# bifurcationkit/BifurcationKit.jl

Measured on NVIDIA H100. Metric: continuation steps/sec (SH2d PALC), higher is better.
Workload: dtype f64

## Files before the change

### bifurcationkit.jl_b200/csrc/bk_common.cuh

```cuda
#pragma once
#include <cuda_runtime.h>
#include <stdint.h>
#include <stdlib.h>
#include <string>
#include <unordered_map>
#include <vector>
#include "../../include/bk200.h"
#include <nvtx3/nvToolsExt.h>

struct BkRange {
  explicit BkRange(const char* name) { nvtxRangePushA(name); }
  ~BkRange() { nvtxRangePop(); }
};

#define BK_MAX_PAR 8
#define BK_NSM_FALLBACK 132

struct OpDesc {
  int kind;
  int nx, ny, nz;
  double cx, cy, cz;
  double par[BK_MAX_PAR];
  const double* u;
  double a0, a1;
// ... 76 lines not shown
      cudaEvent_t a, b;
      cudaEventCreate(&a);
      cudaEventCreate(&b);
      pairs.push_back({a, b});
    }
    cudaEventRecord(pairs[used++].first, st);
  }
  void end(cudaStream_t st) { cudaEventRecord(pairs[used - 1].second, st); }
  long long harvest(double& ms) {
    long long k = 0;
    for (size_t i = 0; i < used; ++i) {
      float t = 0;
      if (cudaEventElapsedTime(&t, pairs[i].first, pairs[i].second) == cudaSuccess) {
        ms += t;
        ++k;
      }
    }
    used = 0;
    return k;
  }
  void destroy() {
    for (auto& p : pairs) {
      cudaEventDestroy(p.first);
      cudaEventDestroy(p.second);
    }
    pairs.clear();
    used = 0;
  }
};

struct bk_ctx {
  int device = 0;
  int nsm = BK_NSM_FALLBACK;
  cudaStream_t stream = nullptr;
  int kind = 0;
  long long dims[3] = {1, 1, 1};
  double lengths[3] = {1, 1, 1};
  double par[BK_MAX_PAR] = {0};
  long long N = 0;
  long long N0 = 0;
  bool cplx = false;
  double shift_imag = 0;
  bool transpose = false;
  int m = 0;
  long long ld = 0;
  double* u_state = nullptr;
  double jpar[BK_MAX_PAR] = {0};
  bool have_state = false;
  double* phi = nullptr;
  double* xpi = nullptr;
  double* fcache = nullptr;
  double phi_dot_xpi = 0;
  double* V = nullptr;
  double* w = nullptr;
  double* z = nullptr;
  double* r = nullptr;
  double* scales = nullptr;
  double* gcoef = nullptr;
  double* hcols = nullptr;
  double* hcols2 = nullptr;
  double* h_pinned = nullptr;
  double* partials = nullptr;
  int gmax = 0;
  unsigned int* counters = nullptr;
  double* red_out = nullptr;
  double* red_pinned = nullptr;
// ... 54 lines not shown
  return g < c->gmax ? g : c->gmax;
}
static inline double bk_inv_h2(const bk_ctx* c, int d) {
  const double h = 2 * c->lengths[d] / c->dims[d];
  return 1.0 / (h * h);
}

bool bk_is_device_ptr(const void* p);
int bk_stage_in(bk_ctx* c, const double* p, long long n, int slot, bool copy_in, double** dev);
int bk_stage_out(bk_ctx* c, double* p, long long n, const double* dev);

OpDesc bk_make_op(bk_ctx* c, double a0, double a1);
OpDesc bk_make_residual_op(bk_ctx* c);
int bk_launch_residual(bk_ctx* c, const double* u_dev, double* out_dev);
int bk_launch_apply(bk_ctx* c, const OpDesc& op, const double* in_dev, const double* in_scale_ptr, double* out_dev);
int bk_potrap_refresh_cache(bk_ctx* c);

int bk_precond_apply_dev(bk_ctx* c, const double* in_dev, double* out_dev, long long n);

int bk_periodic_setup(bk_ctx* c);
int bk_periodic_residual(bk_ctx* c, const OpDesc& op, const double* u, double* out);
int bk_periodic_jvp(bk_ctx* c, const OpDesc& op, const double* in, const double* sp, double* out);
int bk_periodic_fused(bk_ctx* c, const OpDesc& op, const double* in, const double* sp, double* out, bool left);

int bk_dev_axpby(bk_ctx* c, double* y, double a, const double* x, double b, long long n);
int bk_dev_scale(bk_ctx* c, double* x, double a, long long n);
int bk_dev_dot(bk_ctx* c, const double* x, const double* y, long long n, double* out_host);
int bk_dev_norminf(bk_ctx* c, const double* x, long long n, double* out_host);
int bk_dev_copy(bk_ctx* c, double* dst, const double* src, long long n);

int bk_gmres_dev(bk_ctx* c, const OpDesc& op, const double* rhs_dev, double* x_dev, const bk_gmres_opts* o,
                 int* converged, int* iters, double* resnorm);
int bk_launch_dots(bk_ctx* c, const double* basis, const double* scales, const double* w, long long n, int j, double* hcol,
                   double* gcoef);
int bk_launch_update(bk_ctx* c, const double* basis, const double* gcoef, const double* w, long long n, int j, double* vout,
                     double* h_out, double* scale_out);
int bk_launch_lincomb(bk_ctx* c, const double* basis, const double* scales, double* x, double beta, long long n, int k,
                      const double* coef_dev);
int bk_tmp(bk_ctx* c, int slot, double** out);

void bk_grant_smem(int device, const void* kern, size_t bytes);
template <typename K>
static inline void bk_ensure_smem(bk_ctx* c, K kern, size_t bytes) {
  size_t& cur = c->smem_attr[(const void*)kern];
  if (bytes > cur) {
    bk_grant_smem(c->device, (const void*)kern, bytes);
    cur = bytes;
  }
}

#ifdef __CUDACC__
template <typename... KArgs, typename... Args>
static inline cudaError_t bk_launch_pdl(void (*kern)(KArgs...), dim3 grid, dim3 block, size_t smem, cudaStream_t st, bool pdl,
                                        Args&&... args) {
  cudaLaunchConfig_t cfg = {};
  cfg.gridDim = grid;
  cfg.blockDim = block;
  cfg.dynamicSmemBytes = smem;
  cfg.stream = st;
  cudaLaunchAttribute at[1];
  at[0].id = cudaLaunchAttributeProgrammaticStreamSerialization;
  at[0].val.programmaticStreamSerializationAllowed = 1;
  cfg.attrs = at;
  static int no_pdl = -1;
  if (no_pdl < 0) no_pdl = getenv("BK_NO_PDL") ? 1 : 0;
  cfg.numAttrs = pdl && !no_pdl ? 1 : 0;
  return cudaLaunchKernelEx(&cfg, kern, KArgs(args)...);
}
template <typename... KArgs, typename... Args>
// ... 89 lines not shown
```

### bifurcationkit.jl_b200/csrc/bk_ctx.cu

```cuda
#include <cstdio>
#include <cstring>
#include <map>
#include <mutex>
#include <new>
#include "bk_common.cuh"

int bk_fail(bk_ctx* c, int code, const char* what, const char* file, int line) {
  if (c) {
    char buf[512];
    snprintf(buf, sizeof buf, "%s (%s:%d)", what, file, line);
    c->err = buf;
  }
  return code;
}

void bk_grant_smem(int device, const void* kern, size_t bytes) {
  static std::mutex mu;
  static std::map<std::pair<int, const void*>, size_t> granted;
  std::lock_guard<std::mutex> lk(mu);
  size_t& cur = granted[{device, kern}];
  if (bytes <= cur) return;
  cudaFuncSetAttribute(kern, cudaFuncAttributeMaxDynamicSharedMemorySize, (int)bytes);
  if (bytes > 48 * 1024) cudaFuncSetAttribute(kern, cudaFuncAttributePreferredSharedMemoryCarveout, 100);
  cur = bytes;
// ... 63 lines not shown
  if (!c) return BK_ERR_ARG;
  *out = c;
  c->device = device;
  c->cplx = (kind & BK_COMPLEX) != 0;
  kind &= ~BK_COMPLEX;
  c->kind = kind;
  for (int i = 0; i < 3; ++i) {
    c->dims[i] = dims ? (dims[i] > 0 ? dims[i] : 1) : 1;
    c->lengths[i] = lengths ? lengths[i] : 1.0;
  }
  const BkKindTraits* kt = bk_kind_traits(kind);
  if (!kt) return bk_fail(c, BK_ERR_ARG, "unknown problem kind", __FILE__, __LINE__);
  if (kt->pow2_grid)
    for (int d = 0; d < 2; ++d) {
      const long long v = c->dims[d];
      BK_CHECK(c, v >= 64 && v <= 2048 && (v & (v - 1)) == 0,
               "BK_SH2D_PERIODIC: Nx and Ny must be powers of two from 64 to 2048");
    }
  long long n = kt->fields;
  for (int d = 0; d < kt->ndims; ++d) n *= c->dims[d];
  n += kt->extra;
  BK_CHECK(c, n >= 2, "problem too small");
  BK_CHECK(c, krylov_m >= 1 && krylov_m <= 1024, "krylov_m out of range");
  BK_CHECK(c, !c->cplx || kt->complex_ok, "BK_COMPLEX is not available for the periodic-orbit functional");
  c->N0 = n;
  if (c->cplx) n *= 2;
  c->N = n;
  c->m = krylov_m;
  c->ld = ((n + 2 + 31) / 32) * 32;
  BK_CUDA(c, cudaSetDevice(device));
  cudaDeviceProp prop;
  BK_CUDA(c, cudaGetDeviceProperties(&prop, device));
  c->nsm = prop.multiProcessorCount;
  if (const char* e = getenv("BK_NSM")) {
    const int v = atoi(e);
    if (v >= 1 && v <= 1024) c->nsm = v;
  }
  BK_CUDA(c, cudaStreamCreateWithFlags(&c->stream, cudaStreamNonBlocking));
  size_t ld = (size_t)c->ld, m = (size_t)c->m;
  BK_CUDA(c, cudaMalloc(&c->u_state, 8 * ld));
  BK_CUDA(c, cudaMalloc(&c->V, 8 * ld * (m + 1)));
  BK_CUDA(c, cudaMalloc(&c->w, 8 * ld));
  BK_CUDA(c, cudaMalloc(&c->z, 8 * ld));
  BK_CUDA(c, cudaMalloc(&c->r, 8 * ld));
  BK_CUDA(c, cudaMemset(c->u_state, 0, 8 * ld));
  BK_CUDA(c, cudaMemset(c->V, 0, 8 * ld * (m + 1)));
  BK_CUDA(c, cudaMemset(c->w, 0, 8 * ld));
  BK_CUDA(c, cudaMemset(c->z, 0, 8 * ld));
  BK_CUDA(c, cudaMemset(c->r, 0, 8 * ld));
  BK_CUDA(c, cudaMalloc(&c->scales, 8 * (m + 4)));
  BK_CUDA(c, cudaMalloc(&c->gcoef, 8 * (m + 4)));
  BK_CUDA(c, cudaMalloc(&c->hcols, 8 * (m + 1) * (m + 4)));
  BK_CUDA(c, cudaMalloc(&c->hcols2, 8 * (m + 1) * (m + 4)));
  BK_CUDA(c, cudaMemset(c->hcols, 0, 8 * (m + 1) * (m + 4)));
  BK_CUDA(c, cudaMemset(c->hcols2, 0, 8 * (m + 1) * (m + 4)));
  BK_CUDA(c, cudaMallocHost(&c->h_pinned, 2 * 8 * (m + 1) * (m + 4)));
  long long g = (n + 2 + 255) / 256 + 8;
  if (kind == BK_SH2D) {
    long long gf = ((c->dims[0] + 255) / 256) * c->dims[1] + 8;
    if (gf > g) g = gf;
  }
  if (g < 4 * c->nsm) g = 4 * c->nsm;
  c->gmax = (int)g;
  BK_CUDA(c, cudaMalloc(&c->partials, 8 * (m + 4) * (size_t)c->gmax));
  BK_CUDA(c, cudaMalloc(&c->counters, 64 * sizeof(unsigned int)));
  BK_CUDA(c, cudaMemset(c->counters, 0, 64 * sizeof(unsigned int)));
// ... 261 lines not shown
```

### bifurcationkit.jl_b200/csrc/bk_eigs.cu

```cuda
#include <algorithm>
#include <cmath>
#include <complex>
#include <vector>
#include "bk_common.cuh"

typedef std::complex<double> cplx;

static bool hess_eigvals(const std::vector<double>& Hr, int n, int ldh, std::vector<cplx>& ev) {
  std::vector<cplx> A((size_t)n * n);
  for (int j = 0; j < n; ++j)
    for (int i = 0; i < n; ++i) A[i + (size_t)j * n] = (i <= j + 1) ? cplx(Hr[i + (size_t)j * ldh], 0.0) : cplx(0, 0);
  ev.assign(n, cplx(0, 0));
  int hi = n - 1, iter = 0;
  const double eps = 2.2e-16;
  std::vector<cplx> cs(n), sn(n);
  while (hi >= 0) {
    if (hi == 0) {
      ev[0] = A[0];
      break;
    }
    int l = hi;
    while (l > 0) {
      double s = std::abs(A[(l - 1) + (size_t)(l - 1) * n]) + std::abs(A[l + (size_t)l * n]);
      if (s == 0.0) s = 1.0;
// ... 161 lines not shown
          S[k + (size_t)q * n] = sn * skp + cs * skq;
        }
      }
  }
  w.resize(n);
  for (int i = 0; i < n; ++i) w[i] = A[i + (size_t)i * n];
}

static __global__ void k_fill_ones(double* p, int n) {
  int i = blockIdx.x * blockDim.x + threadIdx.x;
  if (i < n) p[i] = 1.0;
}
static __global__ void k_start_vector(double* v, long long n) {
  for (long long i = (long long)blockIdx.x * blockDim.x + threadIdx.x; i < n; i += (long long)gridDim.x * blockDim.x) {
    unsigned long long z = (unsigned long long)i * 0x9E3779B97F4A7C15ULL + 0x1234567ULL;
    z = (z ^ (z >> 30)) * 0xBF58476D1CE4E5B9ULL;
    z = (z ^ (z >> 27)) * 0x94D049BB133111EBULL;
    z ^= z >> 31;
    v[i] = (double)(z >> 11) * (1.0 / 9007199254740992.0) + 0.05;
  }
}

struct EigWork {
  int S;
  double* ones;
  double* hA;
  double* hB;
  double* gco;
  double* coef;
  double* hp;
};

static int arnoldi_start(bk_ctx* c, const EigWork& ws, const double* x, long long n) {
  BK_TRY(bk_launch_update(c, c->Q, ws.gco, x, n, 0, c->Q, ws.hA, ws.hB));
  BK_CUDA(c, cudaMemcpyAsync(ws.hp, ws.hA, 8, cudaMemcpyDeviceToHost, c->stream));
  BK_CUDA(c, cudaStreamSynchronize(c->stream));
  BK_CHECK(c, ws.hp[0] > 0, "zero start vector");
  BK_TRY(bk_dev_scale(c, c->Q, 1.0 / ws.hp[0], n));
  return BK_OK;
}

static int arnoldi_expand(bk_ctx* c, const EigWork& ws, const OpDesc& op, const bk_gmres_opts* inner, double* x, long long n,
                          int m, int kstart, std::vector<double>& H, int* keff, int* nops) {
  const int S = ws.S;
  *keff = m;
  for (int k = kstart; k < m; ++k) {
    const int j = k + 1;
    int cv = 0, it = 0;
    int st = bk_gmres_dev(c, op, c->Q + (size_t)k * c->ld, x, inner, &cv, &it, nullptr);
    if (st < 0) return st;
    ++*nops;
    double* qn = c->Q + (size_t)(k + 1) * c->ld;
    BK_TRY(bk_launch_dots(c, c->Q, ws.ones, x, n, j, ws.hA, ws.gco));
    BK_TRY(bk_launch_update(c, c->Q, ws.gco, x, n, j, qn, ws.hA + j, ws.hB + S - 1));
    BK_TRY(bk_launch_dots(c, c->Q, ws.ones, qn, n, j, ws.hB, ws.gco));
    BK_TRY(bk_launch_update(c, c->Q, ws.gco, qn, n, j, qn, ws.hA + j, ws.hB + S - 1));
    BK_CUDA(c, cudaMemcpyAsync(ws.hp, ws.hA, 8 * (size_t)(2 * S), cudaMemcpyDeviceToHost, c->stream));
    BK_CUDA(c, cudaStreamSynchronize(c->stream));
    const double* hp = ws.hp;
    double cn = 0;
    for (int i = 0; i < j; ++i) {
      H[i + (size_t)k * (m + 1)] = hp[i] + hp[S + i];
      cn = fmax(cn, fabs(H[i + (size_t)k * (m + 1)]));
    }
    double hk1 = hp[j];
    H[j + (size_t)k * (m + 1)] = hk1;
    if (!(hk1 > 1e-14 * fmax(cn, 1e-300))) {
      *keff = k + 1;
      return BK_OK;
    }
    BK_TRY(bk_dev_scale(c, qn, 1.0 / hk1, n));
  }
  return BK_OK;
}

extern "C" int32_t bk_eigs_shift_invert(bk_ctx* c, double sigma, int32_t nev, int32_t krylovdim, double tol,
                                        int32_t maxrestart, const bk_gmres_opts* inner, const double* v0, double* vals_re,
                                        double* vals_im, double* vecs, int32_t* nconv, int32_t* nops) {
  BK_ENTER(c);
  BkRange nvtx_range("bk_eigs_shift_invert");
  BK_CHECK(c, c->have_state, "bk_jac_set_state must be called first");
  BK_CHECK(c, inner != nullptr && vals_re && vals_im, "null argument");
  const long long n = c->N;
  int m = krylovdim;
  if ((long long)m > n) m = (int)n;
  BK_CHECK(c, nev >= 1 && nev <= m, "need 1 <= nev <= krylovdim <= N");
  if (maxrestart < 1) maxrestart = 1;
  if (c->qcap < m) {
    BK_CUDA(c, cudaStreamSynchronize(c->stream));
// ... 168 lines not shown
```

### bifurcationkit.jl_b200/csrc/bk_krylov.cu

```cuda
#include <cmath>
#include <cstdlib>
#include <cstring>
#include <vector>
#include "bk_common.cuh"
#include "bk_stencil.cuh"
#include "bk_krylov_tma.cuh"

static __global__ void __launch_bounds__(BK_THREADS) k_lincomb(double* __restrict__ x, double beta, long long n,
                                                               const double* __restrict__ V, long long ld, int k,
                                                               const double* __restrict__ coef,
                                                               const double* __restrict__ scales) {
  const long long base = (long long)blockIdx.x * BK_TILE;
  double val[BK_EPT];
  int off[BK_EPT];
  bool ok[BK_EPT];
#pragma unroll
  for (int e = 0; e < BK_EPT; ++e) {
    long long g = base + threadIdx.x + e * BK_THREADS;
    ok[e] = g < n;
    off[e] = ok[e] ? (int)g : 0;
    val[e] = (ok[e] && beta != 0.0) ? beta * x[g] : 0.0;
  }
  for (int i = 0; i < k; ++i) {
    const double ci = coef[i] * (scales ? scales[i] : 1.0);
    const double* Vi = V + (long long)i * ld;
#pragma unroll
    for (int e = 0; e < BK_EPT; ++e) val[e] = fma(ci, __ldg(Vi + off[e]), val[e]);
  }
#pragma unroll
  for (int e = 0; e < BK_EPT; ++e)
    if (ok[e]) x[off[e]] = val[e];
}
// ... 47 lines not shown
  p.sred_off = (int)(lo / sizeof(double));
  p.smem = lo + sred;
  return p;
}
static size_t sh2_scratch_bytes(int E) { return sizeof(double) * (size_t)((BK2_ROW + 4) * (E + 4) + (BK2_ROW + 2) * (E + 2)); }

#define BK2_DISPATCH(E, ...) \
  switch (E) {                \
    case 1: { constexpr int EE = 1; __VA_ARGS__; } break; \
    case 2: { constexpr int EE = 2; __VA_ARGS__; } break; \
    case 3: { constexpr int EE = 3; __VA_ARGS__; } break; \
    case 4: { constexpr int EE = 4; __VA_ARGS__; } break; \
    case 5: { constexpr int EE = 5; __VA_ARGS__; } break; \
    case 6: { constexpr int EE = 6; __VA_ARGS__; } break; \
    case 7: { constexpr int EE = 7; __VA_ARGS__; } break; \
    default: { constexpr int EE = 8; __VA_ARGS__; } break; \
  }

static bool fuses_jvp(const bk_ctx* c, const OpDesc& op, const bk_gmres_opts* o) {
  const bool left = o->pc_side == BK_SIDE_LEFT && c->pc.kind != BK_PC_NONE;
  return o->fused && op.kind == BK_SH2D && op.nx % 2 == 0 && !op.cplx && op.bordered <= 1 && !left;
}

static bool fuses_pc(const bk_ctx* c, const OpDesc& op, const bk_gmres_opts* o) {
  const bool side = o->pc_side == BK_SIDE_LEFT || o->pc_side == BK_SIDE_RIGHT;
  return o->fused && op.kind == BK_SH2D_PERIODIC && c->pc.kind == BK_PC_SH_FFT && side && op.bordered == 0 && !op.cplx;
}

static int launch_fused(bk_ctx* c, const OpDesc& op, const double* in, const double* sp, double* w, int j, double* hcol) {
  const int tiles_x = (op.nx + BK2_ROW - 1) / BK2_ROW;
  Plan2 p = plan2(c, (long long)tiles_x * op.ny, sh2_scratch_bytes);
  p.grid = tiles_x * ((op.ny + p.E - 1) / p.E);
  BK_CHECK(c, p.grid <= c->gmax, "partial-sum workspace too small for the fused grid");
  BK2_DISPATCH(p.E, {
    auto kern = op.bordered ? k2_fused<EE, true> : k2_fused<EE, false>;
    return bk_launch(c, kern, dim3(p.grid), dim3(BK2_THREADS), p.smem, op, in, sp, w, c->V, c->ld, j, c->scales, c->partials,
                     c->counters + 0, hcol, c->gcoef, p.NS, p.sred_off);
  });
}

static inline int chunk_grid(long long n) { return (int)((n + BK_TILE - 1) / BK_TILE); }

int bk_launch_dots(bk_ctx* c, const double* basis, const double* scales, const double* w, long long n, int j, double* hcol,
                   double* gcoef) {
  Plan2 p = plan2(c, (n + BK2_ROW - 1) / BK2_ROW, nullptr);
  BK_CHECK(c, p.grid <= c->gmax, "partial-sum workspace too small");
  BK2_DISPATCH(p.E, return bk_launch(c, k2_dots<EE>, dim3(p.grid), dim3(BK2_THREADS), p.smem, w, n, basis, c->ld, j, scales,
                                     c->partials, c->counters + 1, hcol, gcoef, p.NS, p.sred_off));
}
static int launch_dots(bk_ctx* c, const double* w, long long n, int j, double* hcol) {
  return bk_launch_dots(c, c->V, c->scales, w, n, j, hcol, c->gcoef);
}

int bk_launch_update(bk_ctx* c, const double* basis, const double* gcoef, const double* w, long long n, int j, double* vout,
                     double* h_out, double* scale_out) {
  Plan2 p = plan2(c, (n + BK2_ROW - 1) / BK2_ROW, nullptr);
  BK_CHECK(c, p.grid <= c->gmax, "partial-sum workspace too small");
  BK2_DISPATCH(p.E, return bk_launch(c, k2_update<EE>, dim3(p.grid), dim3(BK2_THREADS), p.smem, w, n, basis, c->ld, j, gcoef, vout,
                                     c->partials, c->counters + 2, h_out, scale_out, p.NS));
}
static int launch_update(bk_ctx* c, const double* w, long long n, int j, double* vout, double* h_out, double* scale_out) {
  return bk_launch_update(c, c->V, c->gcoef, w, n, j, vout, h_out, scale_out);
}

int bk_launch_lincomb(bk_ctx* c, const double* basis, const double* scales, double* x, double beta, long long n, int k,
                      const double* coef_dev) {
  return bk_launch_ordered(c, k_lincomb, chunk_grid(n), BK_THREADS, 0, x, beta, n, basis, c->ld, k, coef_dev, scales);
}
static int launch_lincomb(bk_ctx* c, double* x, double beta, long long n, int k, const double* coef_dev, bool use_scales) {
  return bk_launch_lincomb(c, c->V, use_scales ? c->scales : nullptr, x, beta, n, k, coef_dev);
}

static int arnoldi_step(bk_ctx* c, const OpDesc& op, const bk_gmres_opts* o, long long n, int k, bool fuse, bool fuse_pc) {
  const int j = k + 1;
  const int mh = c->m + 4;
  double* hcol = c->h_pinned + (size_t)k * mh;
  double* hcol2 = c->h_pinned + (size_t)(c->m + 1) * mh + (size_t)k * mh;
  const double* in = c->V + (size_t)k * c->ld;
  const double* sp = c->scales + k;
  const bool left = o->pc_side == BK_SIDE_LEFT && c->pc.kind != BK_PC_NONE;
  const bool right = o->pc_side == BK_SIDE_RIGHT && c->pc.kind != BK_PC_NONE;
  if (right && !fuse_pc) {
    BK_TRY(bk_precond_apply_dev(c, in, c->z, n));
    in = c->z;
  }
  const bool timed = c->timing_now;
  const double* wfin = c->w;
  if (fuse_pc) {
    BK_TRY(bk_periodic_fused(c, op, in, sp, c->w, left));
  } else if (!fuse) {
    BK_TRY(bk_launch_apply(c, op, in, sp, c->w));
    if (left) {
      BK_TRY(bk_precond_apply_dev(c, c->w, c->r, n));
      wfin = c->r;
    }
  }
  if (timed) c->fused_timer.begin(c->stream);
  BK_TRY(fuse ? launch_fused(c, op, in, sp, c->w, j, hcol) : launch_dots(c, wfin, n, j, hcol));
  if (timed) c->fused_timer.end(c->stream);
  double* vnext = c->V + (size_t)(k + 1) * c->ld;
  if (timed) c->fused_timer.begin(c->stream);
  BK_TRY(launch_update(c, wfin, n, j, vnext, hcol + j, c->scales + k + 1));
  if (timed) c->fused_timer.end(c->stream);
  if (o->orth == BK_ORTH_CGS2) {
    BK_TRY(launch_dots(c, vnext, n, j, hcol2));
    BK_TRY(launch_update(c, vnext, n, j, vnext, hcol + j, c->scales + k + 1));
  }
  BK_CUDA(c, cudaEventRecord(c->events[k], c->stream));
  const long long step_bytes = 8LL * n * (2LL * j + 4) + (op.bordered ? 16LL * n : 0LL);
  c->stats.last_fused_bytes += step_bytes;
  c->stats.last_fused_launches += 2;
  if (fuse && (c->timing_now || !c->timing)) {
    c->stats.total_fused_bytes += step_bytes;
    c->stats.total_fused_launches += 2;
  }
  return BK_OK;
}

static int init_residual(bk_ctx* c, const OpDesc& op, const bk_gmres_opts* o, long long n, const double* rhs, const double* x,
                         bool x_zero, double* beta) {
  const bool left = o->pc_side == BK_SIDE_LEFT && c->pc.kind != BK_PC_NONE;
  const double* r = rhs;
  if (!x_zero) {
    BK_TRY(bk_launch_apply(c, op, x, nullptr, c->w));
    BK_TRY(bk_dev_axpby(c, c->w, 1.0, rhs, -1.0, n));
    r = c->w;
  }
  if (left) {
    BK_TRY(bk_precond_apply_dev(c, r, c->r, n));
    r = c->r;
  }
  BK_TRY(launch_update(c, r, n, 0, c->V, c->red_out, c->scales));
  BK_CUDA(c, cudaMemcpyAsync(c->red_pinned, c->red_out, 8, cudaMemcpyDeviceToHost, c->stream));
  BK_CUDA(c, cudaStreamSynchronize(c->stream));
  *beta = c->red_pinned[0];
  return BK_OK;
}

int bk_gmres_dev(bk_ctx* c, const OpDesc& op, const double* rhs, double* x, const bk_gmres_opts* o, int* converged,
                 int* iters, double* resnorm) {
  const long long n = op.N + op.bordered;
  BK_CHECK(c, n <= c->ld, "system larger than the context");
  BK_CHECK(c, (n % 2 == 0) || n + 1 <= c->ld, "no pad element left for an odd-sized bordered system");
  int restart = o->restart;
  if (restart > c->m) restart = c->m;
  if ((long long)restart > n) restart = (int)n;
  BK_CHECK(c, restart >= 1, "restart must be >= 1");
  const int maxiter = o->maxiter;
  const int mh = c->m + 4;
  const bool right = o->pc_side == BK_SIDE_RIGHT && c->pc.kind != BK_PC_NONE;
  BK_CHECK(c, o->pc_side == BK_SIDE_NONE || c->pc.kind != BK_PC_NONE, "pc_side set but no preconditioner was set up");
  const bool fuse = fuses_jvp(c, op, o);
  const bool fuse_pc = fuses_pc(c, op, o);
  c->stats.last_fused_bytes = 0;
  c->stats.last_fused_launches = 0;
  c->stats.last_fused_ms = 0.0;
  c->solve_count++;
  c->timing_now = c->timing && (c->solve_count % c->timing_every == 0);
  c->fused_timer.used = 0;

  BK_CUDA(c, cudaMemsetAsync(x, 0, 8 * (size_t)n, c->stream));
  bool x_zero = true;
  int total = 0;
  bool conv = false;
  double tol = 0.0, res = 0.0;
// ... 160 lines not shown
```

### bifurcationkit.jl_b200/csrc/bk_krylov_tma.cuh

```cuda
#pragma once
#include "bk_common.cuh"
#include "bk_async.cuh"

#define BK2_CONS 256
#define BK2_THREADS 288
#define BK2_EMAX 8
#define BK2_ROW 256

struct Tile2 {
  long long base;
  int rs;
  int rows;
  int len;
  int last_len;
};

#define BK2_MAXSTAGES 8
struct Ring {
  unsigned long long full[BK2_MAXSTAGES];
  unsigned long long empty[BK2_MAXSTAGES];
};

__device__ __forceinline__ void ring_init(Ring* rg, int NS) {
  if (threadIdx.x == 0) {
    for (int s = 0; s < NS; ++s) {
      mbar_init(&rg->full[s], 1);
      mbar_init(&rg->empty[s], 8);
    }
    fence_mbar_init();
  }
}

template <int E, int MODE, bool REV = false>
__device__ __forceinline__ void stream_basis(const Tile2& tl, const double* __restrict__ V, long long ld, int j, double* ring,
                                             int NS, Ring* rg, double (&val)[E], double* sred,
                                             const double* __restrict__ gcoef) {
  const int warp = threadIdx.x >> 5, lane = threadIdx.x & 31;
  if (warp == 8) {
    if (lane == 0) {
      fence_proxy_async_smem();
      const unsigned row_b = (unsigned)(((tl.len + 1) & ~1) * 8);
      const unsigned last_b = (unsigned)(((tl.last_len + 1) & ~1) * 8);
      const bool contiguous = (tl.rs == BK2_ROW) && (tl.len == BK2_ROW);
      const unsigned total = row_b * (unsigned)(tl.rows - 1) + last_b;
      for (int i = 0; i < j; ++i) {
        const int s = i % NS, round = i / NS;
        if (round > 0) mbar_wait(&rg->empty[s], (unsigned)((round - 1) & 1));
        mbar_arrive_expect_tx(&rg->full[s], total);
        const double* src = V + (long long)(REV ? j - 1 - i : i) * ld + tl.base;
        double* dst = ring + (size_t)s * (E * BK2_ROW);
        if (contiguous) {
          bulk_g2s(dst, src, total, &rg->full[s]);
        } else {
          for (int r = 0; r < tl.rows - 1; ++r) bulk_g2s(dst + r * BK2_ROW, src + (long long)r * tl.rs, row_b, &rg->full[s]);
          bulk_g2s(dst + (tl.rows - 1) * BK2_ROW, src + (long long)(tl.rows - 1) * tl.rs, last_b, &rg->full[s]);
        }
      }
    }
  } else {
    const int t = threadIdx.x;
    if (MODE == 0) {
      for (int i = 0; i < j; i += 2) {
        const int s0 = i % NS, s1 = (i + 1) % NS;
        const bool two = (i + 1 < j);
        mbar_wait(&rg->full[s0], (unsigned)((i / NS) & 1));
        const double* st0 = ring + (size_t)s0 * (E * BK2_ROW) + t;
        double a0 = 0.0, a1 = 0.0;
#pragma unroll
        for (int e = 0; e < E; ++e) {
          const int lim = (e == tl.rows - 1) ? tl.last_len : tl.len;
          if (e < tl.rows && t < lim) a0 = fma(st0[e * BK2_ROW], val[e], a0);
        }
        if (two) {
          mbar_wait(&rg->full[s1], (unsigned)(((i + 1) / NS) & 1));
          const double* st1 = ring + (size_t)s1 * (E * BK2_ROW) + t;
#pragma unroll
          for (int e = 0; e < E; ++e) {
            const int lim = (e == tl.rows - 1) ? tl.last_len : tl.len;
            if (e < tl.rows && t < lim) a1 = fma(st1[e * BK2_ROW], val[e], a1);
          }
        }
        consumer_release_fence();
        __syncwarp();
        if (lane == 0) {
          mbar_arrive(&rg->empty[s0]);
          if (two) mbar_arrive(&rg->empty[s1]);
        }
#pragma unroll
        for (int o = 16; o > 0; o >>= 1) {
          a0 += __shfl_xor_sync(0xffffffffu, a0, o);
          a1 += __shfl_xor_sync(0xffffffffu, a1, o);
        }
        if (lane == 0) {
          sred[i * 8 + warp] = a0;
          if (two) sred[(i + 1) * 8 + warp] = a1;
        }
      }
    } else {
      for (int i = 0; i < j; ++i) {
        const int s = i % NS;
        mbar_wait(&rg->full[s], (unsigned)((i / NS) & 1));
        const double* st = ring + (size_t)s * (E * BK2_ROW) + t;
        const double g = __ldg(gcoef + (REV ? j - 1 - i : i));
#pragma unroll
        for (int e = 0; e < E; ++e) {
          const int lim = (e == tl.rows - 1) ? tl.last_len : tl.len;
          if (e < tl.rows && t < lim) val[e] = fma(-g, st[e * BK2_ROW], val[e]);
        }
        consumer_release_fence();
        __syncwarp();
        if (lane == 0) mbar_arrive(&rg->empty[s]);
      }
    }
  }
}

struct BorderFin {
  double bscale, bc, xp;
  double* w_tail;
  const double* V_tail;
  long long ld;
};
__device__ __forceinline__ void dots_finish(int j, const double* sred, const double* __restrict__ scales,
                                            double* __restrict__ partials, unsigned int* counter, double* __restrict__ hcol,
                                            double* __restrict__ gcoef, int* s_flag, const BorderFin* bord = nullptr,
                                            double* s_wp = nullptr) {
  const int G = gridDim.x;
  const int jj = bord ? j + 1 : j;
  for (int i = threadIdx.x; i < jj; i += blockDim.x) {
    double t = 0.0;
#pragma unroll
    for (int k = 0; k < 8; ++k) t += sred[i * 8 + k];
    partials[(long long)i * G + blockIdx.x] = t;
  }
  if (bk_last_block(counter, s_flag)) {
    const int warp = threadIdx.x >> 5, lane = threadIdx.x & 31, nw = blockDim.x >> 5;
    double wp = 0.0;
    if (bord) {
      if (warp == 0) {
        double t = 0.0;
        for (int k = lane; k < G; k += 32) t += __ldcg(partials + (long long)j * G + k);
        t = bk_warp_sum(t);
        if (lane == 0) {
          *s_wp = bord->bscale * t + bord->bc * bord->xp;
          *bord->w_tail = *s_wp;
        }
      }
      __syncthreads();
      wp = *s_wp;
    }
    for (int i = warp; i < j; i += nw) {
      double t = 0.0;
      for (int k = lane; k < G; k += 32) t += __ldcg(partials + (long long)i * G + k);
      t = bk_warp_sum(t);
      if (lane == 0) {
        if (bord) t = fma(__ldg(bord->V_tail + (long long)i * bord->ld), wp, t);
        const double s = scales[i];
        const double h = s * t;
        hcol[i] = h;
        gcoef[i] = h * s;
      }
    }
  }
}

template <int E>
struct Sh2Scratch {
  static constexpr int VX = BK2_ROW + 4, VY = E + 4, QX = BK2_ROW + 2, QY = E + 2;
  static constexpr int V_ELEMS = VX * VY, Q_ELEMS = QX * QY;
  static constexpr size_t BYTES = sizeof(double) * (size_t)(V_ELEMS + Q_ELEMS);
};

template <int E>
__device__ __forceinline__ void sh2_tile_issue(const OpDesc& op, const double* __restrict__ in, int x0, int y0, double* scratch,
                                               unsigned long long* tbar) {
  using S = Sh2Scratch<E>;
  const int nx = op.nx, ny = op.ny;
  const int len = min(BK2_ROW, nx - x0);
  mbar_arrive_expect_tx(tbar, (unsigned)(len * 8) * (unsigned)S::VY);
#pragma unroll 1
  for (int jj = 0; jj < S::VY; ++jj) {
    int gy = y0 - 2 + jj;
    gy = gy < 0 ? 0 : (gy > ny - 1 ? ny - 1 : gy);
    bulk_g2s(scratch + jj * S::VX + 2, in + x0 + (long long)gy * nx, (unsigned)(len * 8), tbar);
  }
}

template <int E, bool BORDERED, bool RESID = false>
__device__ __forceinline__ void sh2_tile_eval(const OpDesc& op, const double* __restrict__ in, double in_scale, int x0, int y0,
                                              double* scratch, unsigned long long* tbar, double (&val)[E], double xp,
                                              double* bsum) {
  using S = Sh2Scratch<E>;
  double* vs = scratch;
  double* qs = scratch + S::V_ELEMS;
// ... 37 lines not shown
      const double c0 = p[0];
      const double l1v = in_scale * (c0 + op.cx * (p[-1] - 2.0 * c0 + p[1]) + op.cy * (p[-S::QX] - 2.0 * c0 + p[S::QX]));
      const double v = in_scale * vs[(t + 2) + (e + 2) * S::VX];
      if (RESID) {
        r = v * (l + v * (nu - v)) - l1v;
      } else {
        const double coef = l + g[e] * (2.0 * nu - 3.0 * g[e]);
        r = op.a0 * v + op.a1 * (coef * v - l1v);
        if (BORDERED) r += op.bshift * v;
      }
    }
    val[e] = r;
  }
  if (BORDERED) {
#pragma unroll
    for (int e = 0; e < E; ++e) g[e] = (colok && e < rows) ? __ldg(op.ba + gx + (long long)(y0 + e) * nx) : 0.0;
#pragma unroll
    for (int e = 0; e < E; ++e) val[e] = fma(xp, g[e], val[e]);
#pragma unroll
    for (int e = 0; e < E; ++e) g[e] = (colok && e < rows) ? __ldg(op.bb + gx + (long long)(y0 + e) * nx) : 0.0;
#pragma unroll
    for (int e = 0; e < E; ++e)
      if (colok && e < rows) *bsum = fma(g[e], in_scale * vs[(t + 2) + (e + 2) * S::VX], *bsum);
  }
}

template <int E, bool BORDERED>
static __global__ void __launch_bounds__(BK2_THREADS, 4) k2_fused(OpDesc op, const double* __restrict__ in,
                                                                  const double* __restrict__ in_scale_ptr,
                                                                  double* __restrict__ w, const double* __restrict__ V,
                                                                  long long ld, int j, const double* __restrict__ scales,
                                                                  double* __restrict__ partials, unsigned int* counter,
                                                                  double* __restrict__ hcol, double* __restrict__ gcoef,
                                                                  int NS, int sred_off) {
  extern __shared__ __align__(128) double smem2[];
  __shared__ Ring rg;
  __shared__ __align__(8) unsigned long long tbar;
  __shared__ int s_flag;
  double* ring = smem2;
  double* sred = smem2 + sred_off;
  if (threadIdx.x == 0) mbar_init(&tbar, 1);
  ring_init(&rg, NS);
  const int tiles_x = (op.nx + BK2_ROW - 1) / BK2_ROW;
  const int x0 = (blockIdx.x % tiles_x) * BK2_ROW, y0 = (blockIdx.x / tiles_x) * E;
  double val[E];
  Tile2 tl;
  tl.base = x0 + (long long)y0 * op.nx;
  tl.rs = op.nx;
  tl.rows = min(E, op.ny - y0);
  tl.len = min(BK2_ROW, op.nx - x0);
  tl.last_len = tl.len;
  __syncthreads();
  bk_pdl_sync();
  const double s = in_scale_ptr ? __ldg(in_scale_ptr) : 1.0;
  if (threadIdx.x == BK2_CONS) {
    sh2_tile_issue<E>(op, in, x0, y0, smem2, &tbar);
    const unsigned row_b = (unsigned)(((tl.len + 1) & ~1) * 8);
    for (int r = 0; r < tl.rows; ++r) {
      const long long o = tl.base + (long long)r * tl.rs;
      bulk_prefetch_l2(op.u + o, row_b);
      if (BORDERED) {
        bulk_prefetch_l2(op.ba + o, row_b);
        bulk_prefetch_l2(op.bb + o, row_b);
      }
    }
    const int npf = j < 2 * NS ? j : 2 * NS;
    for (int i = 0; i < npf; ++i)
      for (int r = 0; r < tl.rows; ++r) bulk_prefetch_l2(V + (long long)i * ld + tl.base + (long long)r * tl.rs, row_b);
  }
  const double xp = BORDERED ? s * __ldg(in + op.N) : 0.0;
  double bsum = 0.0;
  sh2_tile_eval<E, BORDERED>(op, in, s, x0, y0, smem2, &tbar, val, xp, &bsum);
  if (threadIdx.x < tl.len) {
#pragma unroll
    for (int e = 0; e < E; ++e)
      if (e < tl.rows) w[tl.base + (long long)e * tl.rs + threadIdx.x] = val[e];
  }
  fence_proxy_async_smem();
  __syncthreads();
  stream_basis<E, 0>(tl, V, ld, j, ring, NS, &rg, val, sred, nullptr);
  if (BORDERED) {
    __shared__ double s_wp;
    bsum = bk_warp_sum(bsum);
    if ((threadIdx.x & 31) == 0 && threadIdx.x < BK2_CONS) sred[j * 8 + (threadIdx.x >> 5)] = bsum;
    __syncthreads();
    BorderFin bf;
    bf.bscale = op.bscale;
    bf.bc = op.bc;
    bf.xp = xp;
    bf.w_tail = w + op.N;
    bf.V_tail = V + op.N;
    bf.ld = ld;
    dots_finish(j, sred, scales, partials, counter, hcol, gcoef, &s_flag, &bf, &s_wp);
  } else {
    __syncthreads();
    dots_finish(j, sred, scales, partials, counter, hcol, gcoef, &s_flag);
  }
}

template <int E, int MODE>
static __global__ void __launch_bounds__(BK2_THREADS, 4) k2_apply(OpDesc op, const double* __restrict__ in,
                                                                  const double* __restrict__ in_scale_ptr, double* __restrict__ out) {
// ... 15 lines not shown
      for (int r = 0; r < rows; ++r) bulk_prefetch_l2(op.u + x0 + (long long)(y0 + r) * op.nx, row_b);
    }
  }
  double val[E];
  double bsum = 0.0;
  sh2_tile_eval<E, false, MODE == 1>(op, in, s, x0, y0, smem2, &tbar, val, 0.0, &bsum);
  if (threadIdx.x < len) {
#pragma unroll
    for (int e = 0; e < E; ++e)
      if (e < rows) out[x0 + (long long)(y0 + e) * op.nx + threadIdx.x] = val[e];
  }
}

__device__ __forceinline__ Tile2 linear_tile(long long n, int E) {
  Tile2 tl;
  tl.base = (long long)blockIdx.x * (E * BK2_ROW);
  tl.rs = BK2_ROW;
  long long rem = n - tl.base;
  int rows = (int)((rem + BK2_ROW - 1) / BK2_ROW);
  tl.rows = rows < E ? rows : E;
  tl.len = BK2_ROW;
  long long lastrem = rem - (long long)(tl.rows - 1) * BK2_ROW;
  tl.last_len = lastrem < BK2_ROW ? (int)lastrem : BK2_ROW;
  if (tl.rows == 1) tl.len = tl.last_len;
  return tl;
}

template <int E>
static __global__ void __launch_bounds__(BK2_THREADS, 4) k2_dots(const double* __restrict__ w, long long n,
                                                                 const double* __restrict__ V, long long ld, int j,
                                                                 const double* __restrict__ scales,
                                                                 double* __restrict__ partials, unsigned int* counter,
                                                                 double* __restrict__ hcol, double* __restrict__ gcoef, int NS,
                                                                 int sred_off) {
  extern __shared__ __align__(128) double smem2[];
  __shared__ Ring rg;
  __shared__ int s_flag;
  double* ring = smem2;
  double* sred = smem2 + sred_off;
  ring_init(&rg, NS);
  const Tile2 tl = linear_tile(n, E);
  double val[E];
  bk_pdl_sync();
#pragma unroll
  for (int e = 0; e < E; ++e) {
    const int lim = (e == tl.rows - 1) ? tl.last_len : tl.len;
    val[e] = (threadIdx.x < BK2_ROW && e < tl.rows && (int)threadIdx.x < lim) ? w[tl.base + e * BK2_ROW + threadIdx.x] : 0.0;
  }
  __syncthreads();
  stream_basis<E, 0>(tl, V, ld, j, ring, NS, &rg, val, sred, nullptr);
  __syncthreads();
  dots_finish(j, sred, scales, partials, counter, hcol, gcoef, &s_flag);
}

template <int E>
static __global__ void __launch_bounds__(BK2_THREADS, 4) k2_update(const double* w, long long n,
                                                                   const double* __restrict__ V, long long ld, int j,
                                                                   const double* __restrict__ gcoef, double* vout,
                                                                   double* __restrict__ partials, unsigned int* counter,
                                                                   double* __restrict__ h_out, double* __restrict__ scale_out,
                                                                   int NS) {
  extern __shared__ __align__(128) double smem2[];
  __shared__ Ring rg;
  __shared__ double s_w[9];
  __shared__ int s_flag;
  double* ring = smem2;
  ring_init(&rg, NS);
  const Tile2 tl = linear_tile(n, E);
  double val[E];
  const int t = threadIdx.x;
  bk_pdl_sync();
#pragma unroll
  for (int e = 0; e < E; ++e) {
    const int lim = (e == tl.rows - 1) ? tl.last_len : tl.len;
    val[e] = (t < BK2_ROW && e < tl.rows && t < lim) ? w[tl.base + e * BK2_ROW + t] : 0.0;
  }
  __syncthreads();
  stream_basis<E, 1, true>(tl, V, ld, j, ring, NS, &rg, val, nullptr, gcoef);
  double acc = 0.0;
  if (t < BK2_ROW) {
#pragma unroll
    for (int e = 0; e < E; ++e) {
      const int lim = (e == tl.rows - 1) ? tl.last_len : tl.len;
      if (e < tl.rows && t < lim) {
        vout[tl.base + e * BK2_ROW + t] = val[e];
        acc = fma(val[e], val[e], acc);
      }
    }
  }
  acc = bk_warp_sum(acc);
  const int lane = t & 31, wid = t >> 5;
  if (lane == 0) s_w[wid] = acc;
  __syncthreads();
  if (t == 0) {
    double r = 0;
    for (int k = 0; k < 9; ++k) r += s_w[k];
    partials[blockIdx.x] = r;
  }
  if (bk_last_block(counter, &s_flag)) {
    double r = 0.0;
    for (int k = t; k < (int)gridDim.x; k += blockDim.x) r += __ldcg(partials + k);
    r = bk_warp_sum(r);
    if (lane == 0) s_w[wid] = r;
    __syncthreads();
    if (t == 0) {
      double q = 0;
      for (int k = 0; k < 9; ++k) q += s_w[k];
      const double h = sqrt(q);
      *h_out = h;
      *scale_out = 1.0 / h;
    }
// ... 3 lines not shown
```

Baseline: 4.294.

## Issue basis TMA loads before PDL wait and parallelize dot-product reduction

The dots and update kernels now issue the first ring-buffer bulk loads of Krylov basis vectors before the programmatic-dependent-launch wait, so basis streaming overlaps the previous kernel's tail. The fused kernel moves its L2 prefetches ahead of the PDL sync and caps the prefetch count by a fraction of L2 size. The last-block reduction in dots_finish folds partial rows with wider, prefetch-unrolled loads into shared memory, then applies scales in parallel across threads. The basis vectors are not written by the preceding kernel, so the early loads are intended to be safe, but this relies on that ordering assumption holding.

New measurement: 4.364 (median of 6 runs). +1.6%, better.

```diff
diff --git a/bifurcationkit.jl_b200/csrc/bk_common.cuh b/bifurcationkit.jl_b200/csrc/bk_common.cuh
--- a/bifurcationkit.jl_b200/csrc/bk_common.cuh
+++ b/bifurcationkit.jl_b200/csrc/bk_common.cuh
@@ -132,6 +132,7 @@
 struct bk_ctx {
   int device = 0;
   int nsm = BK_NSM_FALLBACK;
+  long long l2_bytes = 0;
   cudaStream_t stream = nullptr;
   int kind = 0;
   long long dims[3] = {1, 1, 1};
@@ -252,9 +253,9 @@
 int bk_gmres_dev(bk_ctx* c, const OpDesc& op, const double* rhs_dev, double* x_dev, const bk_gmres_opts* o,
                  int* converged, int* iters, double* resnorm);
 int bk_launch_dots(bk_ctx* c, const double* basis, const double* scales, const double* w, long long n, int j, double* hcol,
-                   double* gcoef);
+                   double* gcoef, bool prewait);
 int bk_launch_update(bk_ctx* c, const double* basis, const double* gcoef, const double* w, long long n, int j, double* vout,
-                     double* h_out, double* scale_out);
+                     double* h_out, double* scale_out, bool prewait);
 int bk_launch_lincomb(bk_ctx* c, const double* basis, const double* scales, double* x, double beta, long long n, int k,
                       const double* coef_dev);
 int bk_tmp(bk_ctx* c, int slot, double** out);
diff --git a/bifurcationkit.jl_b200/csrc/bk_ctx.cu b/bifurcationkit.jl_b200/csrc/bk_ctx.cu
--- a/bifurcationkit.jl_b200/csrc/bk_ctx.cu
+++ b/bifurcationkit.jl_b200/csrc/bk_ctx.cu
@@ -119,6 +119,7 @@
   cudaDeviceProp prop;
   BK_CUDA(c, cudaGetDeviceProperties(&prop, device));
   c->nsm = prop.multiProcessorCount;
+  c->l2_bytes = prop.l2CacheSize;
   if (const char* e = getenv("BK_NSM")) {
     const int v = atoi(e);
     if (v >= 1 && v <= 1024) c->nsm = v;
diff --git a/bifurcationkit.jl_b200/csrc/bk_eigs.cu b/bifurcationkit.jl_b200/csrc/bk_eigs.cu
--- a/bifurcationkit.jl_b200/csrc/bk_eigs.cu
+++ b/bifurcationkit.jl_b200/csrc/bk_eigs.cu
@@ -217,7 +217,7 @@
 };
 
 static int arnoldi_start(bk_ctx* c, const EigWork& ws, const double* x, long long n) {
-  BK_TRY(bk_launch_update(c, c->Q, ws.gco, x, n, 0, c->Q, ws.hA, ws.hB));
+  BK_TRY(bk_launch_update(c, c->Q, ws.gco, x, n, 0, c->Q, ws.hA, ws.hB, false));
   BK_CUDA(c, cudaMemcpyAsync(ws.hp, ws.hA, 8, cudaMemcpyDeviceToHost, c->stream));
   BK_CUDA(c, cudaStreamSynchronize(c->stream));
   BK_CHECK(c, ws.hp[0] > 0, "zero start vector");
@@ -236,10 +236,10 @@
     if (st < 0) return st;
     ++*nops;
     double* qn = c->Q + (size_t)(k + 1) * c->ld;
-    BK_TRY(bk_launch_dots(c, c->Q, ws.ones, x, n, j, ws.hA, ws.gco));
-    BK_TRY(bk_launch_update(c, c->Q, ws.gco, x, n, j, qn, ws.hA + j, ws.hB + S - 1));
-    BK_TRY(bk_launch_dots(c, c->Q, ws.ones, qn, n, j, ws.hB, ws.gco));
-    BK_TRY(bk_launch_update(c, c->Q, ws.gco, qn, n, j, qn, ws.hA + j, ws.hB + S - 1));
+    BK_TRY(bk_launch_dots(c, c->Q, ws.ones, x, n, j, ws.hA, ws.gco, false));
+    BK_TRY(bk_launch_update(c, c->Q, ws.gco, x, n, j, qn, ws.hA + j, ws.hB + S - 1, false));
+    BK_TRY(bk_launch_dots(c, c->Q, ws.ones, qn, n, j, ws.hB, ws.gco, false));
+    BK_TRY(bk_launch_update(c, c->Q, ws.gco, qn, n, j, qn, ws.hA + j, ws.hB + S - 1, false));
     BK_CUDA(c, cudaMemcpyAsync(ws.hp, ws.hA, 8 * (size_t)(2 * S), cudaMemcpyDeviceToHost, c->stream));
     BK_CUDA(c, cudaStreamSynchronize(c->stream));
     const double* hp = ws.hp;
diff --git a/bifurcationkit.jl_b200/csrc/bk_krylov.cu b/bifurcationkit.jl_b200/csrc/bk_krylov.cu
--- a/bifurcationkit.jl_b200/csrc/bk_krylov.cu
+++ b/bifurcationkit.jl_b200/csrc/bk_krylov.cu
@@ -1,3 +1,4 @@
+#include <algorithm>
 #include <cmath>
 #include <cstdlib>
 #include <cstring>
@@ -111,35 +112,38 @@
   Plan2 p = plan2(c, (long long)tiles_x * op.ny, sh2_scratch_bytes);
   p.grid = tiles_x * ((op.ny + p.E - 1) / p.E);
   BK_CHECK(c, p.grid <= c->gmax, "partial-sum workspace too small for the fused grid");
+  const long long l2_vecs = std::max(1LL, c->l2_bytes / 4 / (8LL * (op.N + op.bordered)));
+  const int npf = (int)std::min({(long long)j, 2LL * p.NS, l2_vecs});
   BK2_DISPATCH(p.E, {
     auto kern = op.bordered ? k2_fused<EE, true> : k2_fused<EE, false>;
     return bk_launch(c, kern, dim3(p.grid), dim3(BK2_THREADS), p.smem, op, in, sp, w, c->V, c->ld, j, c->scales, c->partials,
-                     c->counters + 0, hcol, c->gcoef, p.NS, p.sred_off);
+                     c->counters + 0, hcol, c->gcoef, p.NS, p.sred_off, npf);
   });
 }
 
 static inline int chunk_grid(long long n) { return (int)((n + BK_TILE - 1) / BK_TILE); }
 
 int bk_launch_dots(bk_ctx* c, const double* basis, const double* scales, const double* w, long long n, int j, double* hcol,
-                   double* gcoef) {
+                   double* gcoef, bool prewait) {
   Plan2 p = plan2(c, (n + BK2_ROW - 1) / BK2_ROW, nullptr);
   BK_CHECK(c, p.grid <= c->gmax, "partial-sum workspace too small");
   BK2_DISPATCH(p.E, return bk_launch(c, k2_dots<EE>, dim3(p.grid), dim3(BK2_THREADS), p.smem, w, n, basis, c->ld, j, scales,
-                                     c->partials, c->counters + 1, hcol, gcoef, p.NS, p.sred_off));
-}
-static int launch_dots(bk_ctx* c, const double* w, long long n, int j, double* hcol) {
-  return bk_launch_dots(c, c->V, c->scales, w, n, j, hcol, c->gcoef);
+                                     c->partials, c->counters + 1, hcol, gcoef, p.NS, p.sred_off, prewait ? 1 : 0));
+}
+static int launch_dots(bk_ctx* c, const double* w, long long n, int j, double* hcol, bool prewait) {
+  return bk_launch_dots(c, c->V, c->scales, w, n, j, hcol, c->gcoef, prewait);
 }
 
 int bk_launch_update(bk_ctx* c, const double* basis, const double* gcoef, const double* w, long long n, int j, double* vout,
-                     double* h_out, double* scale_out) {
+                     double* h_out, double* scale_out, bool prewait) {
   Plan2 p = plan2(c, (n + BK2_ROW - 1) / BK2_ROW, nullptr);
   BK_CHECK(c, p.grid <= c->gmax, "partial-sum workspace too small");
   BK2_DISPATCH(p.E, return bk_launch(c, k2_update<EE>, dim3(p.grid), dim3(BK2_THREADS), p.smem, w, n, basis, c->ld, j, gcoef, vout,
-                                     c->partials, c->counters + 2, h_out, scale_out, p.NS));
-}
-static int launch_update(bk_ctx* c, const double* w, long long n, int j, double* vout, double* h_out, double* scale_out) {
-  return bk_launch_update(c, c->V, c->gcoef, w, n, j, vout, h_out, scale_out);
+                                     c->partials, c->counters + 2, h_out, scale_out, p.NS, prewait ? 1 : 0));
+}
+static int launch_update(bk_ctx* c, const double* w, long long n, int j, double* vout, double* h_out, double* scale_out,
+                         bool prewait) {
+  return bk_launch_update(c, c->V, c->gcoef, w, n, j, vout, h_out, scale_out, prewait);
 }
 
 int bk_launch_lincomb(bk_ctx* c, const double* basis, const double* scales, double* x, double beta, long long n, int k,
@@ -175,15 +179,15 @@
     }
   }
   if (timed) c->fused_timer.begin(c->stream);
-  BK_TRY(fuse ? launch_fused(c, op, in, sp, c->w, j, hcol) : launch_dots(c, wfin, n, j, hcol));
+  BK_TRY(fuse ? launch_fused(c, op, in, sp, c->w, j, hcol) : launch_dots(c, wfin, n, j, hcol, true));
   if (timed) c->fused_timer.end(c->stream);
   double* vnext = c->V + (size_t)(k + 1) * c->ld;
   if (timed) c->fused_timer.begin(c->stream);
-  BK_TRY(launch_update(c, wfin, n, j, vnext, hcol + j, c->scales + k + 1));
+  BK_TRY(launch_update(c, wfin, n, j, vnext, hcol + j, c->scales + k + 1, true));
   if (timed) c->fused_timer.end(c->stream);
   if (o->orth == BK_ORTH_CGS2) {
-    BK_TRY(launch_dots(c, vnext, n, j, hcol2));
-    BK_TRY(launch_update(c, vnext, n, j, vnext, hcol + j, c->scales + k + 1));
+    BK_TRY(launch_dots(c, vnext, n, j, hcol2, true));
+    BK_TRY(launch_update(c, vnext, n, j, vnext, hcol + j, c->scales + k + 1, true));
   }
   BK_CUDA(c, cudaEventRecord(c->events[k], c->stream));
   const long long step_bytes = 8LL * n * (2LL * j + 4) + (op.bordered ? 16LL * n : 0LL);
@@ -209,7 +213,7 @@
     BK_TRY(bk_precond_apply_dev(c, r, c->r, n));
     r = c->r;
   }
-  BK_TRY(launch_update(c, r, n, 0, c->V, c->red_out, c->scales));
+  BK_TRY(launch_update(c, r, n, 0, c->V, c->red_out, c->scales, false));
   BK_CUDA(c, cudaMemcpyAsync(c->red_pinned, c->red_out, 8, cudaMemcpyDeviceToHost, c->stream));
   BK_CUDA(c, cudaStreamSynchronize(c->stream));
   *beta = c->red_pinned[0];
diff --git a/bifurcationkit.jl_b200/csrc/bk_krylov_tma.cuh b/bifurcationkit.jl_b200/csrc/bk_krylov_tma.cuh
--- a/bifurcationkit.jl_b200/csrc/bk_krylov_tma.cuh
+++ b/bifurcationkit.jl_b200/csrc/bk_krylov_tma.cuh
@@ -31,31 +31,45 @@
   }
 }
 
+template <int E, bool REV>
+__device__ __forceinline__ void ring_issue(const Tile2& tl, const double* __restrict__ V, long long ld, int j, double* ring,
+                                           int NS, Ring* rg, int i) {
+  const unsigned row_b = (unsigned)(((tl.len + 1) & ~1) * 8);
+  const unsigned last_b = (unsigned)(((tl.last_len + 1) & ~1) * 8);
+  const bool contiguous = (tl.rs == BK2_ROW) && (tl.len == BK2_ROW);
+  const unsigned total = row_b * (unsigned)(tl.rows - 1) + last_b;
+  const int s = i % NS, round = i / NS;
+  if (round > 0) mbar_wait(&rg->empty[s], (unsigned)((round - 1) & 1));
+  mbar_arrive_expect_tx(&rg->full[s], total);
+  const double* src = V + (long long)(REV ? j - 1 - i : i) * ld + tl.base;
+  double* dst = ring + (size_t)s * (E * BK2_ROW);
+  if (contiguous) {
+    bulk_g2s(dst, src, total, &rg->full[s]);
+  } else {
+    for (int r = 0; r < tl.rows - 1; ++r) bulk_g2s(dst + r * BK2_ROW, src + (long long)r * tl.rs, row_b, &rg->full[s]);
+    bulk_g2s(dst + (tl.rows - 1) * BK2_ROW, src + (long long)(tl.rows - 1) * tl.rs, last_b, &rg->full[s]);
+  }
+}
+
+template <int E, bool REV>
+__device__ __forceinline__ int ring_issue_prewait(const Tile2& tl, const double* __restrict__ V, long long ld, int j,
+                                                  double* ring, int NS, Ring* rg) {
+  const int n = j < NS ? j : NS;
+  __syncthreads();
+  if (threadIdx.x == BK2_CONS)
+    for (int i = 0; i < n; ++i) ring_issue<E, REV>(tl, V, ld, j, ring, NS, rg, i);
+  return n;
+}
+
 template <int E, int MODE, bool REV = false>
 __device__ __forceinline__ void stream_basis(const Tile2& tl, const double* __restrict__ V, long long ld, int j, double* ring,
                                              int NS, Ring* rg, double (&val)[E], double* sred,
-                                             const double* __restrict__ gcoef) {
+                                             const double* __restrict__ gcoef, int issued = 0) {
   const int warp = threadIdx.x >> 5, lane = threadIdx.x & 31;
   if (warp == 8) {
     if (lane == 0) {
       fence_proxy_async_smem();
-      const unsigned row_b = (unsigned)(((tl.len + 1) & ~1) * 8);
-      const unsigned last_b = (unsigned)(((tl.last_len + 1) & ~1) * 8);
-      const bool contiguous = (tl.rs == BK2_ROW) && (tl.len == BK2_ROW);
-      const unsigned total = row_b * (unsigned)(tl.rows - 1) + last_b;
-      for (int i = 0; i < j; ++i) {
-        const int s = i % NS, round = i / NS;
-        if (round > 0) mbar_wait(&rg->empty[s], (unsigned)((round - 1) & 1));
-        mbar_arrive_expect_tx(&rg->full[s], total);
-        const double* src = V + (long long)(REV ? j - 1 - i : i) * ld + tl.base;
-        double* dst = ring + (size_t)s * (E * BK2_ROW);
-        if (contiguous) {
-          bulk_g2s(dst, src, total, &rg->full[s]);
-        } else {
-          for (int r = 0; r < tl.rows - 1; ++r) bulk_g2s(dst + r * BK2_ROW, src + (long long)r * tl.rs, row_b, &rg->full[s]);
-          bulk_g2s(dst + (tl.rows - 1) * BK2_ROW, src + (long long)(tl.rows - 1) * tl.rs, last_b, &rg->full[s]);
-        }
-      }
+      for (int i = issued; i < j; ++i) ring_issue<E, REV>(tl, V, ld, j, ring, NS, rg, i);
     }
   } else {
     const int t = threadIdx.x;
@@ -121,7 +135,21 @@
   const double* V_tail;
   long long ld;
 };
-__device__ __forceinline__ void dots_finish(int j, const double* sred, const double* __restrict__ scales,
+#define BK2_FOLD_PF 16
+__device__ __forceinline__ double fold_row(const double* __restrict__ row, int G, int lane) {
+  double t = 0.0;
+  for (int k0 = lane; k0 < G; k0 += 32 * BK2_FOLD_PF) {
+    double x[BK2_FOLD_PF];
+#pragma unroll
+    for (int q = 0; q < BK2_FOLD_PF; ++q) x[q] = (k0 + 32 * q < G) ? __ldcg(row + k0 + 32 * q) : 0.0;
+#pragma unroll
+    for (int q = 0; q < BK2_FOLD_PF; ++q)
+      if (k0 + 32 * q < G) t += x[q];
+  }
+  return bk_warp_sum(t);
+}
+
+__device__ __forceinline__ void dots_finish(int j, double* sred, const double* __restrict__ scales,
                                             double* __restrict__ partials, unsigned int* counter, double* __restrict__ hcol,
                                             double* __restrict__ gcoef, int* s_flag, const BorderFin* bord = nullptr,
                                             double* s_wp = nullptr) {
@@ -135,31 +163,29 @@
   }
   if (bk_last_block(counter, s_flag)) {
     const int warp = threadIdx.x >> 5, lane = threadIdx.x & 31, nw = blockDim.x >> 5;
-    double wp = 0.0;
-    if (bord) {
-      if (warp == 0) {
-        double t = 0.0;
-        for (int k = lane; k < G; k += 32) t += __ldcg(partials + (long long)j * G + k);
-        t = bk_warp_sum(t);
-        if (lane == 0) {
-          *s_wp = bord->bscale * t + bord->bc * bord->xp;
+    const int i0 = threadIdx.x;
+    const double s0 = i0 < j ? scales[i0] : 0.0;
+    const double vt0 = (bord && i0 < j) ? __ldg(bord->V_tail + (long long)i0 * bord->ld) : 0.0;
+    for (int r = warp; r < jj; r += nw) {
+      const double t = fold_row(partials + (long long)r * G, G, lane);
+      if (lane == 0) {
+        if (r == j) {
+          *s_wp = fma(bord->bc, bord->xp, bord->bscale * t);
           *bord->w_tail = *s_wp;
-        }
-      }
-      __syncthreads();
-      wp = *s_wp;
-    }
-    for (int i = warp; i < j; i += nw) {
-      double t = 0.0;
-      for (int k = lane; k < G; k += 32) t += __ldcg(partials + (long long)i * G + k);
-      t = bk_warp_sum(t);
-      if (lane == 0) {
-        if (bord) t = fma(__ldg(bord->V_tail + (long long)i * bord->ld), wp, t);
-        const double s = scales[i];
-        const double h = s * t;
-        hcol[i] = h;
-        gcoef[i] = h * s;
-      }
+        } else {
+          sred[r] = t;
+        }
+      }
+    }
+    __syncthreads();
+    const double wp = bord ? *s_wp : 0.0;
+    for (int i = threadIdx.x; i < j; i += blockDim.x) {
+      double t = sred[i];
+      if (bord) t = fma(i == i0 ? vt0 : __ldg(bord->V_tail + (long long)i * bord->ld), wp, t);
+      const double s = i == i0 ? s0 : scales[i];
+      const double h = s * t;
+      hcol[i] = h;
+      gcoef[i] = h * s;
     }
   }
 }
@@ -263,7 +289,7 @@
                                                                   long long ld, int j, const double* __restrict__ scales,
                                                                   double* __restrict__ partials, unsigned int* counter,
                                                                   double* __restrict__ hcol, double* __restrict__ gcoef,
-                                                                  int NS, int sred_off) {
+                                                                  int NS, int sred_off, int npf) {
   extern __shared__ __align__(128) double smem2[];
   __shared__ Ring rg;
   __shared__ __align__(8) unsigned long long tbar;
@@ -281,11 +307,7 @@
   tl.rows = min(E, op.ny - y0);
   tl.len = min(BK2_ROW, op.nx - x0);
   tl.last_len = tl.len;
-  __syncthreads();
-  bk_pdl_sync();
-  const double s = in_scale_ptr ? __ldg(in_scale_ptr) : 1.0;
   if (threadIdx.x == BK2_CONS) {
-    sh2_tile_issue<E>(op, in, x0, y0, smem2, &tbar);
     const unsigned row_b = (unsigned)(((tl.len + 1) & ~1) * 8);
     for (int r = 0; r < tl.rows; ++r) {
       const long long o = tl.base + (long long)r * tl.rs;
@@ -295,10 +317,13 @@
         bulk_prefetch_l2(op.bb + o, row_b);
       }
     }
-    const int npf = j < 2 * NS ? j : 2 * NS;
     for (int i = 0; i < npf; ++i)
       for (int r = 0; r < tl.rows; ++r) bulk_prefetch_l2(V + (long long)i * ld + tl.base + (long long)r * tl.rs, row_b);
   }
+  __syncthreads();
+  bk_pdl_sync();
+  const double s = in_scale_ptr ? __ldg(in_scale_ptr) : 1.0;
+  if (threadIdx.x == BK2_CONS) sh2_tile_issue<E>(op, in, x0, y0, smem2, &tbar);
   const double xp = BORDERED ? s * __ldg(in + op.N) : 0.0;
   double bsum = 0.0;
   sh2_tile_eval<E, BORDERED>(op, in, s, x0, y0, smem2, &tbar, val, xp, &bsum);
@@ -380,7 +405,7 @@
                                                                  const double* __restrict__ scales,
                                                                  double* __restrict__ partials, unsigned int* counter,
                                                                  double* __restrict__ hcol, double* __restrict__ gcoef, int NS,
-                                                                 int sred_off) {
+                                                                 int sred_off, int prewait) {
   extern __shared__ __align__(128) double smem2[];
   __shared__ Ring rg;
   __shared__ int s_flag;
@@ -389,6 +414,7 @@
   ring_init(&rg, NS);
   const Tile2 tl = linear_tile(n, E);
   double val[E];
+  const int issued = prewait ? ring_issue_prewait<E, false>(tl, V, ld, j, ring, NS, &rg) : 0;
   bk_pdl_sync();
 #pragma unroll
   for (int e = 0; e < E; ++e) {
@@ -396,7 +422,7 @@
     val[e] = (threadIdx.x < BK2_ROW && e < tl.rows && (int)threadIdx.x < lim) ? w[tl.base + e * BK2_ROW + threadIdx.x] : 0.0;
   }
   __syncthreads();
-  stream_basis<E, 0>(tl, V, ld, j, ring, NS, &rg, val, sred, nullptr);
+  stream_basis<E, 0>(tl, V, ld, j, ring, NS, &rg, val, sred, nullptr, issued);
   __syncthreads();
   dots_finish(j, sred, scales, partials, counter, hcol, gcoef, &s_flag);
 }
@@ -407,7 +433,7 @@
                                                                    const double* __restrict__ gcoef, double* vout,
                                                                    double* __restrict__ partials, unsigned int* counter,
                                                                    double* __restrict__ h_out, double* __restrict__ scale_out,
-                                                                   int NS) {
+                                                                   int NS, int prewait) {
   extern __shared__ __align__(128) double smem2[];
   __shared__ Ring rg;
   __shared__ double s_w[9];
@@ -417,6 +443,7 @@
   const Tile2 tl = linear_tile(n, E);
   double val[E];
   const int t = threadIdx.x;
+  const int issued = prewait ? ring_issue_prewait<E, true>(tl, V, ld, j, ring, NS, &rg) : 0;
   bk_pdl_sync();
 #pragma unroll
   for (int e = 0; e < E; ++e) {
@@ -424,7 +451,7 @@
     val[e] = (t < BK2_ROW && e < tl.rows && t < lim) ? w[tl.base + e * BK2_ROW + t] : 0.0;
   }
   __syncthreads();
-  stream_basis<E, 1, true>(tl, V, ld, j, ring, NS, &rg, val, nullptr, gcoef);
+  stream_basis<E, 1, true>(tl, V, ld, j, ring, NS, &rg, val, nullptr, gcoef, issued);
   double acc = 0.0;
   if (t < BK2_ROW) {
 #pragma unroll
```
